# samiazirar/mvtracker

Hardware: AMD Instinct MI355X
Metric: query-points*frames/sec, 4-view 24-frame 512x512 @1024 queries (higher is better)
Workload: dtype bf16; 1 GPU; c3: 4-view synthetic 24-frame 512x512, 1024 queries, bf16 (configs[2], the metric's config); 4-view 24-frame 512x512, 1024 queries per GPU, corr K=16 x 4 levels, iters=4, 3 windows, random-init weights (seeded recipe); queries_total=1024, parallelism=query-shard x1, frame_store=bf16 rows

## Files before the change

### mvtracker_amd/csrc/block_fused.hip

```cpp
#include "common.h"
#include <stdlib.h>

namespace {

typedef __bf16 bf16x8 __attribute__((ext_vector_type(8)));
typedef __bf16 bf16x4 __attribute__((ext_vector_type(4)));
typedef unsigned u32x4 __attribute__((ext_vector_type(4)));
typedef unsigned u32x2 __attribute__((ext_vector_type(2)));

__device__ __forceinline__ void lds_barrier() {
#ifdef MVT_FULL_BARRIERS
  __syncthreads();
#else
  __builtin_amdgcn_fence(__ATOMIC_RELEASE, "workgroup", "local");
  __builtin_amdgcn_s_barrier();
  __builtin_amdgcn_fence(__ATOMIC_ACQUIRE, "workgroup", "local");
#endif
}

constexpr int NT = 512;
constexpr int C = 256;
constexpr int LDX = C + 8;
template <int NMB> struct Cfg {
  static constexpr int BM = 32 * NMB;
  static constexpr int HC = 256;
  static constexpr int JW = HC / 32;
  static constexpr int NM1 = NMB / (8 / JW);
  static constexpr int LDH = HC + 8;
  static constexpr int LDA = 296;
  static_assert(BM * LDA <= 2 * BM * LDH, "attention tile fits the H buffers");
};
constexpr int YLD = 40;
constexpr int FS = 512;

#ifdef MVT_STAMPS
__device__ unsigned long long mvt_stamp_buf[2 * 8 * 64];
#ifndef MVT_STAMP_SEL
#define MVT_STAMP_SEL true
#endif
#ifndef MVT_STAMP_WG1
#define MVT_STAMP_WG1 100
#endif
#define STAMP(i)                                                                                                  \
  do {                                                                                                            \
    __builtin_amdgcn_sched_barrier(0);                                                                            \
    unsigned long long t_;                                                                                        \
    asm volatile("s_memtime %0\n\ts_waitcnt lgkmcnt(0)" : "=s"(t_)::"memory");                                    \
    __builtin_amdgcn_sched_barrier(0);                                                                            \
    if (lane == 0 && MVT_STAMP_SEL && (bx == 0 || bx == MVT_STAMP_WG1) && by == 0 && bz == 0)  \
      mvt_stamp_buf[((bx ? 1 : 0) * 8 + wave) * 64 + (i)] = t_;                                                   \
  } while (0)
#else
#define STAMP(i) \
  do {           \
  } while (0)
#endif

#if defined(MVT_STAMPS) && defined(MVT_ASTAMPS)
#define ASTAMP(i)                                       \
  do {                                                  \
    const int wave = threadIdx.x >> 6;                  \
    const int bx = blockIdx.x, by = blockIdx.y, bz = blockIdx.z; \
    STAMP(i);                                           \
  } while (0)
#else
#define ASTAMP(i) \
  do {            \
  } while (0)
#endif

struct BlockArgs {
  float* x;
  int ldx;
  const float* att;
  int ldatt, Ko;
  const unsigned short* wo;
  const float* bo;
  int ldwo;
  const unsigned short* w1;
  const float* b1;
  const unsigned short* w2;
  const float* b2;
  int ldw1, ldw2, H;
  mvt_block_next next[MVT_BLOCK_MAX_NEXT];
  int n_next;
  int att_bf16;
  long long M;
  float* ws;
  const unsigned short* aq;
  const unsigned short* ak;
  const unsigned short* av;
  int ldaq, ldakv, S, nkeys, bmv;
  const float* parts;
  int nsplit;
  const float* tokx;
  const unsigned short* win;
  const float* bin;
  const float* virt;
  int ldtok;
  long long Mp;
  const float* t_coords;
  const float* t_fcorr;
  const float* t_ffeats;
  const float* t_maskvis;
  const float* t_pos;
  const float* t_time;
  int t_E, t_Fc, t_Cf, t_D;
  const float* c_ws;
  const float* c_b2;
  float* c_x;
  int c_ldx, c_nch;
  mvt_block_next c_kv;
  mvt_block_next c_next;
};

typedef float f32x2 __attribute__((ext_vector_type(2)));
__device__ __forceinline__ f32x2 gelu_tanh_pk(f32x2 x) {
  const f32x2 c0 = {-2.3022082f, -2.3022082f}, c1 = {-0.10294324f, -0.10294324f}, one = {1.0f, 1.0f};
// ... 304 lines not shown
        }
#pragma unroll
        for (int db = 0; db < 2; ++db) {
          const unsigned short* vr = (db * 32 + r < DHA) ? &vimg[(db * 32 + r) * LDVA + 16 * sk + 4 * h] : zrow + 16 * sk + 4 * h;
          const u32x2 a0 = *reinterpret_cast<const u32x2*>(vr), a1 = *reinterpret_cast<const u32x2*>(vr + 8);
          const bf16x8 va = __builtin_bit_cast(bf16x8, (u32x4){a0[0], a0[1], a1[0], a1[1]});
          oacc[db] = __builtin_amdgcn_mfma_f32_32x32x16_bf16(va, pb, oacc[db], 0, 0, 0);
        }
      }
    }
    __builtin_amdgcn_sched_barrier(0);
    ASTAMP(51 + 2 * mb);
    const float lt = pair_sum(ps);
    const float inv = 1.0f / lt;
    if (qi >= nq) continue;
#pragma unroll
    for (int db = 0; db < 2; ++db) {
#pragma unroll
      for (int gq = 0; gq < 4; ++gq) {
        const int d = db * 32 + 8 * gq + 4 * h;
        if (d < DHA) {
          f32x4 t;
#pragma unroll
          for (int e = 0; e < 4; ++e) t[e] = oacc[db][4 * gq + e] * inv;
          *reinterpret_cast<u32x2*>(&As[(arow0 + qi) * lda + hd * DHA + d]) = __builtin_bit_cast(u32x2, __builtin_convertvector(t, bf16x4));
        }
      }
    }
  }
}

template <int NMB>
__device__ __forceinline__ void ln_to_lds(const f32x16 (&v)[NMB], unsigned short* Xs, float* st, int wave, int lane, float eps,
                                          const float* lnw, const float* lnb, float (&ms)[NMB][2], bool have) {
  constexpr int BM = 32 * NMB;
  const int r = lane & 31, h = lane >> 5;
  f32x4 gw[4], gb[4];
  if (lnw) {
#pragma unroll
    for (int g = 0; g < 4; ++g) {
      gw[g] = *reinterpret_cast<const f32x4*>(lnw + wave * 32 + 8 * g + 4 * h);
      gb[g] = *reinterpret_cast<const f32x4*>(lnb + wave * 32 + 8 * g + 4 * h);
    }
  }
  if (!have) {
#pragma unroll
    for (int mb = 0; mb < NMB; ++mb) {
      float s1 = 0.f, s2 = 0.f;
#pragma unroll
      for (int e = 0; e < 16; ++e) {
        s1 += v[mb][e];
        s2 = fmaf(v[mb][e], v[mb][e], s2);
      }
      s1 += __shfl_xor(s1, 32, 64);
      s2 += __shfl_xor(s2, 32, 64);
      if (h == 0) {
        st[(wave * BM + mb * 32 + r) * 2] = s1;
        st[(wave * BM + mb * 32 + r) * 2 + 1] = s2;
      }
    }
    lds_barrier();
#pragma unroll
    for (int mb = 0; mb < NMB; ++mb) {
      float s1 = 0.f, s2 = 0.f;
#pragma unroll
      for (int w = 0; w < 8; ++w) {
        s1 += st[(w * BM + mb * 32 + r) * 2];
        s2 += st[(w * BM + mb * 32 + r) * 2 + 1];
      }
      const float mean = s1 / (float)C;
      ms[mb][0] = mean;
      ms[mb][1] = fmaxf(s2 / (float)C - mean * mean, 0.f);
    }
  }
#pragma unroll
  for (int mb = 0; mb < NMB; ++mb) {
    const float mean = ms[mb][0];
    const float rstd = 1.0f / sqrtf(ms[mb][1] + eps);
#pragma unroll
    for (int g = 0; g < 4; ++g) {
      const int n = wave * 32 + 8 * g + 4 * h;
      f32x4 o;
#pragma unroll
      for (int e = 0; e < 4; ++e) {
        o[e] = (v[mb][4 * g + e] - mean) * rstd;
        if (lnw) o[e] = o[e] * gw[g][e] + gb[g][e];
      }
      const bf16x4 b = __builtin_convertvector(o, bf16x4);
      *reinterpret_cast<u32x2*>(&Xs[(mb * 32 + r) * LDX + n]) = __builtin_bit_cast(u32x2, b);
    }
  }
  lds_barrier();
}

template <int NMB, int MODE, int ATT>
__global__ __launch_bounds__(NT) void block_fused_bf16(BlockArgs p) {
  using K_ = Cfg<NMB>;
  constexpr int BM = K_::BM, HC = K_::HC, LDH = K_::LDH, LDA = K_::LDA;
  constexpr bool CTX = ATT == 6;
  static_assert(!CTX || (NMB == 2 && MODE == 0), "ATT 6 runs on the 64-row tiles of the point rows");
  constexpr int HSZ = CTX && (64 * LDKV + 1) / 2 > BM * LDH ? (64 * LDKV + 1) / 2 : BM * LDH;
  __shared__ __attribute__((aligned(16))) unsigned short Xs[BM * LDX];
  __shared__ __attribute__((aligned(16))) unsigned short Hs[2][HSZ];
  __shared__ float st[8 * BM * 2];
  __shared__ __attribute__((aligned(16))) float b1s[4 * C];
  __shared__ __attribute__((aligned(16))) float cbs[CTX ? 2 * 288 : 4];

  const int t = threadIdx.x, wave = t >> 6, lane = t & 63;
  const int r = lane & 31, h = lane >> 5;
  int bx = (int)blockIdx.x, by = (int)blockIdx.y, bz = (int)blockIdx.z;
  if constexpr (ATT == 2 || ATT == 3 || ATT == 5 || ATT == 6) {
    const unsigned total = gridDim.x * gridDim.y * gridDim.z;
    if (total % 8 == 0) {
      const unsigned L = blockIdx.x + gridDim.x * (blockIdx.y + gridDim.y * blockIdx.z);
      const unsigned V = (L % 8) * (total / 8) + L / 8;
      bx = (int)(V % gridDim.x);
      by = (int)((V / gridDim.x) % gridDim.y);
      bz = (int)(V / (gridDim.x * gridDim.y));
    }
  }
  static_assert(ATT == 0 || ATT == 5 || MODE != 2, "pass 2 of the split path has no attention");
  static_assert(ATT != 5 || MODE == 2, "ATT 5 = pass 2 on the frame-major tiles of an ATT 2 / ATT 3 pass 1");
  static_assert((MODE != 1 && MODE != 2) || NMB == 1, "the split path runs on 32-row tiles");
  constexpr bool FM = ATT == 2 || ATT == 3 || ATT == 5 || ATT == 6;
  const int bmv = ATT == 1 ? p.bmv : BM;
  const long long m0 = FM ? 0 : (long long)bx * bmv;
  const long long ntok = FM ? p.M / p.S : 0;
  auto grow = [&](int i) -> long long {
    if (FM) {
      const long long tk = (long long)bx * BM + i;
      return tk < ntok ? tk * p.S + (long long)bz : -1;
    }
    const long long m = m0 + i;
    return (i < bmv && m < p.M) ? m : -1;
  };
  const long long rlo = FM ? (long long)bx * BM * p.S : m0;
  const long long rhi = FM ? ((long long)bx * BM + BM) * p.S : m0 + bmv;
  constexpr bool HAS_MLP = MODE == 0 || MODE == 1;
  if (HAS_MLP)
    for (int i = t; i < p.H; i += NT) b1s[i] = p.b1[i];
  const long long ws_tile = FM ? (long long)bz * gridDim.x + bx : (long long)bx;
  const long long ws_ntile = FM ? (long long)gridDim.z * gridDim.x : (long long)gridDim.x;
  auto ws_off = [&](int chunk, int g) -> long long { return ((((long long)chunk * ws_ntile + ws_tile) * 8 + wave) * 4 + g) * 256 + lane * 4; };
  auto active = [&](int q) { return q < p.n_next && rlo < p.next[q].row_hi && rhi > p.next[q].row_lo; };
  bf16x8 wq[PFQ];
  constexpr bool EARLY = NMB == 1 && MODE != 0;
  bool early_have = false;
  const bool outp = MODE != 2 && ATT != 4 && (ATT != 0 || p.att != nullptr);
  const unsigned short* wo_row = p.wo + ((long long)wave * 18 * 64 + lane) * 8;
  const unsigned short* fc1_first = p.w1 + ((long long)(wave % K_::JW) * (C / 16) * 64 + lane) * 8 +
                                    (long long)(MODE == 1 ? by : 0) * K_::JW * (C / 16) * FS;
  auto prefetch_wo = [&]() { fill_wq(wq, wo_row); };
  if (HAS_MLP && !outp) {
    fill_wq(wq, fc1_first);
  } else if (CTX) {
    fill_wq(wq, p.c_kv.w + ((long long)wave * (C / 16) * 64 + lane) * 8);
  } else if (outp) {
    prefetch_wo();
  } else if (EARLY && MODE == 2) {
    const int nb0e = by * 8 + wave;
    if (active(0) && nb0e < (p.next[0].N + 31) / 32) {
      fill_wq(wq, p.next[0].w + ((long long)nb0e * (C / 16) * 64 + lane) * 8);
      early_have = true;
    }
  }

  STAMP(0);
  f32x16 v[NMB];
#pragma unroll
  for (int mb = 0; mb < NMB; ++mb)
#pragma unroll
    for (int e = 0; e < 16; ++e) v[mb][e] = 0.f;

  f32x4 xr[NMB][4];
  auto load_x = [&]() {
    if (ATT == 4 || (MODE == 2 && p.ws)) return;
#pragma unroll
// ... 394 lines not shown
            for (int e = 0; e < 4; ++e) xv[e] += part[mb][g][sidx][e];
          }
#pragma unroll
        for (int e = 0; e < 4; ++e) v[mb][4 * g + e] += xv[e] + p.b2[wave * 32 + 8 * g + 4 * h + e];
      }
  } else if (ATT != 4) {
#pragma unroll
    for (int mb = 0; mb < NMB; ++mb)
#pragma unroll
      for (int g = 0; g < 4; ++g)
#pragma unroll
        for (int e = 0; e < 4; ++e) v[mb][4 * g + e] += xr[mb][g][e];
  }

  auto store_x = [&]() {
#pragma unroll
    for (int mb = 0; mb < NMB; ++mb) {
      const long long m = grow(mb * 32 + r);
      if (m >= 0) {
#pragma unroll
        for (int g = 0; g < 4; ++g) {
          f32x4 o;
#pragma unroll
          for (int e = 0; e < 4; ++e) o[e] = v[mb][4 * g + e];
          *reinterpret_cast<f32x4*>(p.x + m * (long long)p.ldx + wave * 32 + 8 * g + 4 * h) = o;
        }
      }
    }
  };
  STAMP(5);
  float ln_ms[NMB][2];
  if (HAS_MLP) ln_to_lds<NMB>(v, Xs, st, wave, lane, 1e-6f, nullptr, nullptr, ln_ms, false);
  STAMP(6);
  const bool tail_next = MODE == 0 && active(0) && wave < (p.next[0].N + 31) / 32;
  if (HAS_MLP) {
    f32x16 acc2[NMB];
#pragma unroll
    for (int mb = 0; mb < NMB; ++mb)
#pragma unroll
      for (int e = 0; e < 16; ++e) acc2[mb][e] = 0.f;
    constexpr int JW = K_::JW, NM1 = K_::NM1;
    const int jb = wave % JW, mp = wave / JW;
    const int nchunk = p.H / HC;
    const unsigned short* w1row = p.w1 + ((long long)jb * (C / 16) * 64 + lane) * 8;
    const unsigned short* w2row = p.w2 + ((long long)wave * (p.H / 16) * 64 + lane) * 8;
    static_assert(HC / 16 == PFQ && C / 16 == PFQ, "every GEMM segment is exactly one queue length");
    const unsigned short* tail = tail_next ? p.next[0].w + ((long long)wave * (C / 16) * 64 + lane) * 8 : w1row;
    const int c_lo = MODE == 1 ? by : 0, c_hi = MODE == 1 ? c_lo + 1 : nchunk;
#pragma unroll 1
    for (int c = c_lo; c < c_hi; ++c) {
      unsigned short* Hb = Hs[c & 1];
      f32x16 ha[NM1];
#pragma unroll
      for (int i = 0; i < NM1; ++i)
#pragma unroll
        for (int e = 0; e < 16; ++e) ha[i][e] = 0.f;
      STAMP(8 + 5 * c);
      gemm_wq<C / 16, NM1>(ha, wq, w1row + (long long)c * JW * (C / 16) * FS, w2row + (long long)c * (HC / 16) * FS, &Xs[r * LDX + 8 * h], LDX,
                           NM1 * mp);
      STAMP(9 + 5 * c);
#pragma unroll
      for (int i = 0; i < NM1; ++i) {
#pragma unroll
        for (int g = 0; g < 4; ++g) {
          const f32x4 bq = *reinterpret_cast<const f32x4*>(&b1s[c * HC + jb * 32 + 8 * g + 4 * h]);
          f32x4 o;
#ifdef MVT_ABL_NOGELU
#pragma unroll
          for (int e = 0; e < 4; ++e) o[e] = ha[i][4 * g + e] + bq[e];
#else
#pragma unroll
          for (int e = 0; e < 4; e += 2) {
            const f32x2 y = gelu_tanh_pk((f32x2){ha[i][4 * g + e] + bq[e], ha[i][4 * g + e + 1] + bq[e + 1]});
            o[e] = y[0];
            o[e + 1] = y[1];
          }
#endif
          const bf16x4 b = __builtin_convertvector(o, bf16x4);
          *reinterpret_cast<u32x2*>(&Hb[((NM1 * mp + i) * 32 + r) * LDH + jb * 32 + 8 * g + 4 * h]) = __builtin_bit_cast(u32x2, b);
        }
// ... 7 lines not shown
    }
    if (MODE == 1) {
#pragma unroll
      for (int mb = 0; mb < NMB; ++mb) {
        const long long m = grow(mb * 32 + r);
        if (m < 0) continue;
#pragma unroll
        for (int g = 0; g < 4; ++g) {
          f32x4 a4, x4;
#pragma unroll
          for (int e = 0; e < 4; ++e) {
            a4[e] = acc2[mb][4 * g + e];
            x4[e] = v[mb][4 * g + e];
          }
          *reinterpret_cast<f32x4*>(p.ws + ws_off(by + 1, g)) = a4;
          if (by == 0) *reinterpret_cast<f32x4*>(p.ws + ws_off(0, g)) = x4;
        }
      }
      return;
    }
#pragma unroll
    for (int mb = 0; mb < NMB; ++mb)
#pragma unroll
      for (int g = 0; g < 4; ++g)
#pragma unroll
        for (int e = 0; e < 4; ++e) v[mb][4 * g + e] += acc2[mb][4 * g + e] + p.b2[wave * 32 + 8 * g + 4 * h + e];
  }
  STAMP(30);
  if (MODE == 0 || ATT == 4 || (p.ws && by == 0)) store_x();
  STAMP(31);

  bool have = tail_next || early_have;
  bool have_ms = false;
#pragma unroll
  for (int q = 0; q < MVT_BLOCK_MAX_NEXT; ++q) {
    if (q >= p.n_next) break;
    if (!active(q)) continue;
    const mvt_block_next nx = p.next[q];
    lds_barrier();
    for (int i = t; i < nx.N; i += NT) b1s[i] = nx.b[i];
    STAMP(32 + 8 * q);
    ln_to_lds<NMB>(v, Xs, st, wave, lane, nx.eps, nx.lnw, nx.lnb, ln_ms, have_ms);
    have_ms = true;
    STAMP(33 + 8 * q);
    const int nblocks = (nx.N + 31) / 32;
    auto nrow_of = [&](int nb) { return nx.w + ((long long)nb * (C / 16) * 64 + lane) * 8; };
    const int nb0 = MODE == 2 ? by * 8 + wave : wave, nbstep = MODE == 2 ? 8 * (int)gridDim.y : 8;
    if (nb0 < nblocks && !have) fill_wq(wq, nrow_of(nb0));
    const int qn = q + 1 < MVT_BLOCK_MAX_NEXT ? q + 1 : MVT_BLOCK_MAX_NEXT - 1;
    const unsigned short* chain = nullptr;
    if ((MODE == 0 || MODE == 3) && q + 1 < MVT_BLOCK_MAX_NEXT && active(q + 1) && wave < (p.next[qn].N + 31) / 32)
      chain = p.next[qn].w + ((long long)wave * (C / 16) * 64 + lane) * 8;
    have = chain != nullptr && wave < nblocks;
    for (int nb = nb0; nb < nblocks; nb += nbstep) {
      f32x16 acc[NMB];
#pragma unroll
      for (int mb = 0; mb < NMB; ++mb)
#pragma unroll
        for (int e = 0; e < 16; ++e) acc[mb][e] = 0.f;
      gemm_wq<C / 16, NMB>(acc, wq, nrow_of(nb), nb + nbstep < nblocks ? nrow_of(nb + nbstep) : (chain ? chain : nrow_of(nb)), &Xs[r * LDX + 8 * h], LDX, 0);
      STAMP(34 + 8 * q + (nb - nb0) / nbstep);
      if (nx.y_bf16 && nb * 32 + 31 < nx.N && (nx.ldy & 7) == 0 && ((uintptr_t)nx.y & 15) == 0) {
        unsigned short* tile = &Hs[0][0] + wave * (NMB * 32 * YLD);
        __builtin_amdgcn_fence(__ATOMIC_SEQ_CST, "wavefront");
#pragma unroll
        for (int mb = 0; mb < NMB; ++mb)
#pragma unroll
          for (int g = 0; g < 4; ++g) {
            f32x4 o;
// ... 32 lines not shown
        }
      }
    }
    STAMP(39 + 8 * q);
  }
  STAMP(63);
}

__global__ void pack_frag_kernel(const unsigned short* __restrict__ w, int ld, int N, int K, unsigned short* __restrict__ out) {
  const long long total = (long long)((N + 31) / 32) * (K / 16) * 64;
  for (long long i = blockIdx.x * (long long)blockDim.x + threadIdx.x; i < total; i += (long long)gridDim.x * blockDim.x) {
    const int lane = (int)(i & 63);
    const long long f = i >> 6;
    const int ks = (int)(f % (K / 16));
    const int nb = (int)(f / (K / 16));
    const int n = nb * 32 + (lane & 31), k = ks * 16 + 8 * (lane >> 5);
    u32x4 v = (u32x4){0u, 0u, 0u, 0u};
    if (n < N) v = *reinterpret_cast<const u32x4*>(w + (long long)n * ld + k);
    *reinterpret_cast<u32x4*>(out + i * 8) = v;
  }
}

}

#ifdef MVT_STAMPS
extern "C" int mvt_debug_read_stamps(unsigned long long* host) {
  return hipMemcpyFromSymbol(host, HIP_SYMBOL(mvt_stamp_buf), sizeof(unsigned long long) * 2 * 8 * 64) == hipSuccess ? MVT_OK : MVT_ERR_HIP_BASE;
}
extern "C" int mvt_debug_clear_stamps() {
  static unsigned long long z[2 * 8 * 64];
  return hipMemcpyToSymbol(HIP_SYMBOL(mvt_stamp_buf), z, sizeof(z)) == hipSuccess ? MVT_OK : MVT_ERR_HIP_BASE;
}
#endif

extern "C" int mvt_pack_frag_bf16(const unsigned short* w, int ld, int N, int K, unsigned short* out, void* stream) {
  MVT_REQUIRE(w && out && N > 0 && K > 0 && K % 16 == 0 && ld % 8 == 0 && ld >= K);
  MVT_REQUIRE(((uintptr_t)w % 16 == 0) && ((uintptr_t)out % 16 == 0));
  const long long total = (long long)((N + 31) / 32) * (K / 16) * 64;
  hipLaunchKernelGGL(pack_frag_kernel, dim3((unsigned)mvt_cdiv(total, 256)), dim3(256), 0, mvt_stream(stream), w, ld, N, K, out);
  return mvt_launch_status();
}

extern "C" int mvt_block_fused_bf16(float* x, int ldx, const void* att, int att_bf16, int ldatt, int Ko, const unsigned short* wo, int ldwo,
                                    const float* bo, const unsigned short* w1, int ldw1, const float* b1, const unsigned short* w2,
                                    int ldw2, const float* b2, int H, const mvt_block_next* next, int n_next, long long M, int Cc,
                                    float* workspace, void* stream) {
  MVT_REQUIRE(x && w1 && b1 && w2 && b2 && M > 0 && Cc == C && H > 0 && H % 256 == 0 && H <= 4 * C);
  MVT_REQUIRE(ldx % 4 == 0 && ldx >= C);
  MVT_REQUIRE(!att || (wo && bo && Ko == 288 && ldatt % 4 == 0 && ldatt >= Ko));
  MVT_REQUIRE(n_next >= 0 && n_next <= MVT_BLOCK_MAX_NEXT && (n_next == 0 || next));
  MVT_REQUIRE(((uintptr_t)x % 16 == 0) && ((uintptr_t)att % 16 == 0) && ((uintptr_t)wo % 16 == 0) && ((uintptr_t)w1 % 16 == 0) &&
              ((uintptr_t)w2 % 16 == 0));
  BlockArgs a{};
  a.x = x; a.ldx = ldx; a.att = (const float*)att; a.att_bf16 = att_bf16 ? 1 : 0; a.ldatt = ldatt; a.Ko = Ko; a.wo = wo; a.bo = bo; a.ldwo = ldwo;
  a.w1 = w1; a.b1 = b1; a.w2 = w2; a.b2 = b2; a.ldw1 = ldw1; a.ldw2 = ldw2; a.H = H; a.M = M; a.n_next = n_next;
  for (int q = 0; q < n_next; ++q) {
    const mvt_block_next& nx = next[q];
    MVT_REQUIRE(nx.w && nx.b && nx.y && nx.N > 0 && nx.N <= 4 * C && nx.ldy % 4 == 0 && nx.ldy >= nx.N);
    MVT_REQUIRE(nx.y_bf16 == 0 || nx.y_bf16 == 1);
    MVT_REQUIRE((nx.lnw == nullptr) == (nx.lnb == nullptr) && ((uintptr_t)nx.lnw % 16 == 0) && ((uintptr_t)nx.lnb % 16 == 0) && ((uintptr_t)nx.w % 16 == 0) && ((uintptr_t)nx.y % 16 == 0));
    MVT_REQUIRE(nx.row_lo >= 0 && (nx.row_hi == 0 || nx.row_hi > nx.row_lo));
    a.next[q] = nx;
    if (nx.row_hi == 0) a.next[q].row_hi = M;
  }
  static const char* force = getenv("MVT_BLOCK_NMB");
  const int nmb = force ? atoi(force) : (M >= 4096 ? 2 : 1);
  static const bool no_split = getenv("MVT_BLOCK_NOSPLIT") != nullptr;
  a.ws = workspace;
  if (nmb == 2) {
    hipLaunchKernelGGL((block_fused_bf16<2, 0, 0>), dim3((unsigned)mvt_cdiv(M, 64)), dim3(NT), 0, mvt_stream(stream), a);
  } else if (workspace && !no_split && M <= 2048 && M % 32 == 0) {
    MVT_REQUIRE((uintptr_t)workspace % 16 == 0);
    const unsigned tiles = (unsigned)mvt_cdiv(M, 32);
    hipLaunchKernelGGL((block_fused_bf16<1, 1, 0>), dim3(tiles, (unsigned)(H / 256)), dim3(NT), 0, mvt_stream(stream), a);
    int maxblk = 1;
    for (int q = 0; q < n_next; ++q) maxblk = (next[q].N + 31) / 32 > maxblk ? (next[q].N + 31) / 32 : maxblk;
    const unsigned slices = n_next ? (unsigned)mvt_cdiv(maxblk, 8) : 1u;
    hipLaunchKernelGGL((block_fused_bf16<1, 2, 0>), dim3(tiles, slices), dim3(NT), 0, mvt_stream(stream), a);
  } else {
    hipLaunchKernelGGL((block_fused_bf16<1, 0, 0>), dim3((unsigned)mvt_cdiv(M, 32)), dim3(NT), 0, mvt_stream(stream), a);
  }
  return mvt_launch_status();
}

extern "C" int mvt_attn_block_fused_bf16(float* x, int ldx, const mvt_block_attn* attn, const unsigned short* wo, const float* bo,
                                         const unsigned short* w1, const float* b1, const unsigned short* w2, const float* b2, int H,
                                         const mvt_block_next* next, int n_next, long long M, int Cc, float* workspace, void* stream) {
  MVT_REQUIRE(x && attn && wo && bo && w1 && b1 && w2 && b2 && M > 0 && Cc == C && H > 0 && H % 256 == 0 && H <= 4 * C);
  MVT_REQUIRE(ldx % 4 == 0 && ldx >= C && n_next >= 0 && n_next <= MVT_BLOCK_MAX_NEXT && (n_next == 0 || next));
  MVT_REQUIRE(attn->heads == 6 && attn->dim_head == DHA && attn->S >= 1 && M % attn->S == 0);
  MVT_REQUIRE(attn->kind == MVT_ATTN_PARTIALS || (attn->kind == MVT_ATTN_FRAME_CTX && attn->q && attn->ldq % 8 == 0 && attn->ldq >= 288) ||
              (attn->q && attn->k && attn->v && attn->ldq % 8 == 0 && attn->ldkv % 8 == 0 && attn->ldq >= 288 && attn->ldkv >= 288));
  MVT_REQUIRE(((uintptr_t)x % 16 == 0) && ((uintptr_t)wo % 16 == 0) && ((uintptr_t)w1 % 16 == 0) && ((uintptr_t)w2 % 16 == 0));
  MVT_REQUIRE(((uintptr_t)attn->q % 16 == 0) && ((uintptr_t)attn->k % 16 == 0) && ((uintptr_t)attn->v % 16 == 0));
  BlockArgs a{};
  a.x = x; a.ldx = ldx; a.att = nullptr; a.Ko = 288; a.wo = wo; a.bo = bo; a.ldwo = 288;
  a.w1 = w1; a.b1 = b1; a.w2 = w2; a.b2 = b2; a.ldw1 = C; a.ldw2 = H; a.H = H; a.M = M; a.n_next = n_next; a.ws = workspace;
  a.aq = attn->q; a.ak = attn->k; a.av = attn->v; a.ldaq = attn->ldq; a.ldakv = attn->ldkv; a.S = attn->S; a.nkeys = attn->n_keys;
  for (int q = 0; q < n_next; ++q) {
    const mvt_block_next& nx = next[q];
    MVT_REQUIRE(nx.w && nx.b && nx.y && nx.N > 0 && nx.N <= 4 * C && nx.ldy % 4 == 0 && nx.ldy >= nx.N);
    MVT_REQUIRE((nx.y_bf16 == 0 || nx.y_bf16 == 1) && (nx.lnw == nullptr) == (nx.lnb == nullptr) && ((uintptr_t)nx.lnw % 16 == 0) && ((uintptr_t)nx.lnb % 16 == 0));
    MVT_REQUIRE(((uintptr_t)nx.w % 16 == 0) && ((uintptr_t)nx.y % 16 == 0) && nx.row_lo >= 0 && (nx.row_hi == 0 || nx.row_hi > nx.row_lo));
    a.next[q] = nx;
    if (nx.row_hi == 0) a.next[q].row_hi = M;
  }
  const int S = attn->S;
  if (attn->kind == MVT_ATTN_TIME) {
    MVT_REQUIRE(S <= 32 && !workspace);
    static const bool small_tiles = !(getenv("MVT_TIME_NMB1") && atoi(getenv("MVT_TIME_NMB1")) == 0);
    if (small_tiles && mvt_cdiv(M, (32 / S) * S) <= 256) {
      a.bmv = (32 / S) * S;
      hipLaunchKernelGGL((block_fused_bf16<1, 0, 1>), dim3((unsigned)mvt_cdiv(M, a.bmv)), dim3(NT), 0, mvt_stream(stream), a);
      return mvt_launch_status();
    }
    a.bmv = (64 / S) * S;
    hipLaunchKernelGGL((block_fused_bf16<2, 0, 1>), dim3((unsigned)mvt_cdiv(M, a.bmv)), dim3(NT), 0, mvt_stream(stream), a);
  } else if (attn->kind == MVT_ATTN_PARTIALS) {
    MVT_REQUIRE(attn->partials && attn->n_splits >= 1 && attn->n_splits <= MVT_ATTN_NSPLIT && attn->n_keys == 64 && M == 64LL * S);
    MVT_REQUIRE(workspace && (uintptr_t)workspace % 16 == 0 && M <= 2048 && (uintptr_t)attn->partials % 16 == 0);
    a.parts = attn->partials; a.nsplit = attn->n_splits;
    const unsigned tiles = (unsigned)mvt_cdiv(M, 32);
    a.S = S;
    hipLaunchKernelGGL((block_fused_bf16<1, 1, 3>), dim3(2, (unsigned)(H / 256), (unsigned)S), dim3(NT), 0, mvt_stream(stream), a);
    int maxblk = 1;
    for (int q = 0; q < n_next; ++q) maxblk = (next[q].N + 31) / 32 > maxblk ? (next[q].N + 31) / 32 : maxblk;
    const unsigned slices = n_next ? (unsigned)mvt_cdiv(maxblk, 8) : 1u;
    (void)tiles;
    if (!attn->defer_pass2)
      hipLaunchKernelGGL((block_fused_bf16<1, 2, 5>), dim3(2, slices, (unsigned)S), dim3(NT), 0, mvt_stream(stream), a);
  } else if (attn->kind == MVT_ATTN_FRAME) {
    MVT_REQUIRE(attn->n_keys >= 1 && attn->n_keys <= 64);
    const long long ntok = M / S;
    static const bool small_tiles = !(getenv("MVT_FRAME_NMB1") && atoi(getenv("MVT_FRAME_NMB1")) == 0);
    if (ntok * S >= 4096 && small_tiles && mvt_cdiv(ntok, 32) * S <= 256) {
      MVT_REQUIRE(!workspace);
      hipLaunchKernelGGL((block_fused_bf16<1, 0, 2>), dim3((unsigned)mvt_cdiv(ntok, 32), 1, (unsigned)S), dim3(NT), 0, mvt_stream(stream), a);
    } else if (ntok * S >= 4096) {
      MVT_REQUIRE(!workspace);
      hipLaunchKernelGGL((block_fused_bf16<2, 0, 2>), dim3((unsigned)mvt_cdiv(ntok, 64), 1, (unsigned)S), dim3(NT), 0, mvt_stream(stream), a);
    } else {
      MVT_REQUIRE(workspace && (uintptr_t)workspace % 16 == 0 && M <= 2048 && ntok % 32 == 0);
      hipLaunchKernelGGL((block_fused_bf16<1, 1, 2>), dim3((unsigned)(ntok / 32), (unsigned)(H / 256), (unsigned)S), dim3(NT), 0,
                         mvt_stream(stream), a);
      int maxblk = 1;
      for (int q = 0; q < n_next; ++q) maxblk = (next[q].N + 31) / 32 > maxblk ? (next[q].N + 31) / 32 : maxblk;
      const unsigned slices = n_next ? (unsigned)mvt_cdiv(maxblk, 8) : 1u;
      if (!attn->defer_pass2)
        hipLaunchKernelGGL((block_fused_bf16<1, 2, 5>), dim3((unsigned)(ntok / 32), slices, (unsigned)S), dim3(NT), 0, mvt_stream(stream), a);
    }
  } else if (attn->kind == MVT_ATTN_FRAME_CTX) {
    const mvt_block_ctx* cx = attn->ctx;
    const long long ntok = M / S;
    MVT_REQUIRE(cx && attn->n_keys == 64 && ntok * S >= 4096 && !workspace && !attn->defer_pass2);
    MVT_REQUIRE(cx->ws && cx->b2 && cx->x && cx->chunks >= 1 && cx->chunks <= 4 && cx->ldx % 4 == 0 && cx->ldx >= C);
    MVT_REQUIRE(((uintptr_t)cx->ws % 16 == 0) && ((uintptr_t)cx->b2 % 16 == 0) && ((uintptr_t)cx->x % 16 == 0));
    MVT_REQUIRE(cx->kv.w && cx->kv.b && cx->kv.N == 2 * 288 && (cx->kv.lnw == nullptr) == (cx->kv.lnb == nullptr));
    MVT_REQUIRE(((uintptr_t)cx->kv.w % 16 == 0) && ((uintptr_t)cx->kv.lnw % 16 == 0) && ((uintptr_t)cx->kv.lnb % 16 == 0));
    const unsigned tiles = (unsigned)mvt_cdiv(ntok, 64);
    if (cx->next.w) {
      const mvt_block_next& nx = cx->next;
      MVT_REQUIRE(nx.b && nx.y && nx.N > 0 && nx.N <= 4 * C && nx.ldy % 4 == 0 && nx.ldy >= nx.N && (nx.y_bf16 == 0 || nx.y_bf16 == 1));
      MVT_REQUIRE((nx.lnw == nullptr) == (nx.lnb == nullptr) && ((uintptr_t)nx.lnw % 16 == 0) && ((uintptr_t)nx.lnb % 16 == 0));
      MVT_REQUIRE(((uintptr_t)nx.w % 16 == 0) && ((uintptr_t)nx.y % 16 == 0) && (nx.N + 31) / 32 <= 8 * (int)tiles);
    }
    a.c_ws = cx->ws; a.c_b2 = cx->b2; a.c_x = cx->x; a.c_ldx = cx->ldx; a.c_nch = cx->chunks; a.c_kv = cx->kv; a.c_next = cx->next;
    hipLaunchKernelGGL((block_fused_bf16<2, 0, 6>), dim3(tiles, 1, (unsigned)S), dim3(NT), 0, mvt_stream(stream), a);
  } else {
    return MVT_ERR_ARG;
  }
  return mvt_launch_status();
}

extern "C" int mvt_input_proj_bf16(const float* tokens, int ldtok, int token_dim, long long Mp, const unsigned short* win, const float* bin,
                                   const float* virtual_tokens, int S, float* x, int ldx, const mvt_block_next* next, int n_next, long long M,
                                   int Cc, void* stream) {
  MVT_REQUIRE(tokens && win && bin && virtual_tokens && x && next && n_next >= 1 && n_next <= MVT_BLOCK_MAX_NEXT && Cc == C);
  MVT_REQUIRE(M > 0 && Mp >= 0 && Mp <= M && S >= 1 && (M - Mp) % S == 0 && token_dim >= 1 && token_dim <= 37 * 16 && ldtok >= token_dim);
  MVT_REQUIRE(ldtok % 4 == 0 && ldx % 4 == 0 && ldx >= C && ((uintptr_t)tokens % 16 == 0) && ((uintptr_t)win % 16 == 0) && ((uintptr_t)x % 16 == 0));
  BlockArgs a{};
  a.x = x; a.ldx = ldx; a.M = M; a.n_next = n_next; a.H = 4 * C; a.ws = nullptr; a.S = S;
  a.tokx = tokens; a.ldtok = ldtok; a.win = win; a.bin = bin; a.virt = virtual_tokens; a.Mp = Mp;
  for (int q = 0; q < n_next; ++q) {
    const mvt_block_next& nx = next[q];
    MVT_REQUIRE(nx.w && nx.b && nx.y && nx.N > 0 && nx.N <= 4 * C && nx.ldy % 4 == 0 && nx.ldy >= nx.N);
    MVT_REQUIRE((nx.lnw == nullptr) == (nx.lnb == nullptr) && ((uintptr_t)nx.lnw % 16 == 0) && ((uintptr_t)nx.lnb % 16 == 0) && ((uintptr_t)nx.w % 16 == 0) && ((uintptr_t)nx.y % 16 == 0));
    MVT_REQUIRE(nx.row_lo >= 0 && (nx.row_hi == 0 || nx.row_hi > nx.row_lo) && (nx.y_bf16 == 0 || nx.y_bf16 == 1));
    a.next[q] = nx;
    if (nx.row_hi == 0) a.next[q].row_hi = M;
  }
  hipLaunchKernelGGL((block_fused_bf16<2, 3, 4>), dim3((unsigned)mvt_cdiv(M, 64)), dim3(NT), 0, mvt_stream(stream), a);
  return mvt_launch_status();
}

extern "C" int mvt_token_input_proj_bf16(const float* coords, const float* fcorr, int Fc, const float* ffeats, int Cf, const float* mask_vis,
                                         const float* pos, const float* time_embed, int n_tracks, int S, int E,
                                         const unsigned short* win, const float* bin, const float* virtual_tokens, float* x, int ldx,
                                         const mvt_block_next* next, int n_next, long long M, int Cc, void* stream) {
  MVT_REQUIRE(coords && fcorr && ffeats && mask_vis && pos && time_embed && win && bin && virtual_tokens && x && next);
  MVT_REQUIRE(n_next >= 1 && n_next <= MVT_BLOCK_MAX_NEXT && Cc == C && n_tracks > 0 && S >= 1 && E > 0 && E % 2 == 0 && Fc > 0 && Cf > 0);
  const int D = 3 * E + 3 + Fc + Cf + 2;
  const long long Mp = (long long)n_tracks * S;
  MVT_REQUIRE(D <= 37 * 16 && M >= Mp && (M - Mp) % S == 0 && ldx % 4 == 0 && ldx >= C);
  MVT_REQUIRE(((uintptr_t)win % 16 == 0) && ((uintptr_t)x % 16 == 0));
  BlockArgs a{};
  a.x = x; a.ldx = ldx; a.M = M; a.n_next = n_next; a.H = 4 * C; a.ws = nullptr; a.S = S;
  a.tokx = nullptr; a.win = win; a.bin = bin; a.virt = virtual_tokens; a.Mp = Mp;
  a.t_coords = coords; a.t_fcorr = fcorr; a.t_ffeats = ffeats; a.t_maskvis = mask_vis; a.t_pos = pos; a.t_time = time_embed;
  a.t_E = E; a.t_Fc = Fc; a.t_Cf = Cf; a.t_D = D;
  for (int q = 0; q < n_next; ++q) {
    const mvt_block_next& nx = next[q];
    MVT_REQUIRE(nx.w && nx.b && nx.y && nx.N > 0 && nx.N <= 4 * C && nx.ldy % 4 == 0 && nx.ldy >= nx.N);
    MVT_REQUIRE((nx.lnw == nullptr) == (nx.lnb == nullptr) && ((uintptr_t)nx.lnw % 16 == 0) && ((uintptr_t)nx.lnb % 16 == 0) && ((uintptr_t)nx.w % 16 == 0) && ((uintptr_t)nx.y % 16 == 0));
    MVT_REQUIRE(nx.row_lo >= 0 && (nx.row_hi == 0 || nx.row_hi > nx.row_lo) && (nx.y_bf16 == 0 || nx.y_bf16 == 1));
    a.next[q] = nx;
    if (nx.row_hi == 0) a.next[q].row_hi = M;
  }
  hipLaunchKernelGGL((block_fused_bf16<2, 3, 4>), dim3((unsigned)mvt_cdiv(M, 64)), dim3(NT), 0, mvt_stream(stream), a);
  return mvt_launch_status();
}

extern "C" int mvt_ln_proj_bf16(const float* x, int ldx, const mvt_block_next* next, int n_next, long long M, int Cc, void* stream) {
  MVT_REQUIRE(x && next && n_next >= 1 && n_next <= MVT_BLOCK_MAX_NEXT && M > 0 && Cc == C && ldx % 4 == 0 && ldx >= C);
  MVT_REQUIRE((uintptr_t)x % 16 == 0);
  BlockArgs a{};
  a.x = const_cast<float*>(x); a.ldx = ldx; a.M = M; a.n_next = n_next; a.H = 4 * C; a.ws = nullptr;
  int maxblk = 1;
  for (int q = 0; q < n_next; ++q) {
    const mvt_block_next& nx = next[q];
    MVT_REQUIRE(nx.w && nx.b && nx.y && nx.N > 0 && nx.N <= 4 * C && nx.ldy % 4 == 0 && nx.ldy >= nx.N);
    MVT_REQUIRE((nx.lnw == nullptr) == (nx.lnb == nullptr) && ((uintptr_t)nx.lnw % 16 == 0) && ((uintptr_t)nx.lnb % 16 == 0) && ((uintptr_t)nx.w % 16 == 0) && ((uintptr_t)nx.y % 16 == 0));
    MVT_REQUIRE(nx.row_lo >= 0 && (nx.row_hi == 0 || nx.row_hi > nx.row_lo) && (nx.y_bf16 == 0 || nx.y_bf16 == 1));
    a.next[q] = nx;
    if (nx.row_hi == 0) a.next[q].row_hi = M;
    maxblk = (nx.N + 31) / 32 > maxblk ? (nx.N + 31) / 32 : maxblk;
  }
  if (M >= 4096)
    hipLaunchKernelGGL((block_fused_bf16<2, 3, 0>), dim3((unsigned)mvt_cdiv(M, 64)), dim3(NT), 0, mvt_stream(stream), a);
  else
    hipLaunchKernelGGL((block_fused_bf16<1, 2, 0>), dim3((unsigned)mvt_cdiv(M, 32), (unsigned)mvt_cdiv(maxblk, 8)), dim3(NT), 0,
                       mvt_stream(stream), a);
  return mvt_launch_status();
}
```

### mvtracker_amd/csrc/common.h

```cpp
#pragma once
#include <hip/hip_runtime.h>
#include <stdint.h>

#include "../../include/mvtracker_hip.h"

typedef float f32x4 __attribute__((ext_vector_type(4)));
typedef float f32x16 __attribute__((ext_vector_type(16)));

#define MVT_WAVE 64

#define MVT_REQUIRE(cond) \
  do {                    \
    if (!(cond)) return MVT_ERR_ARG; \
  } while (0)

static inline int mvt_launch_status() {
  hipError_t e = hipGetLastError();
  return e == hipSuccess ? MVT_OK : MVT_ERR_HIP_BASE + (int)e;
}

static inline hipStream_t mvt_stream(void* s) { return (hipStream_t)s; }

static inline long long mvt_cdiv(long long a, long long b) { return (a + b - 1) / b; }

__device__ __forceinline__ float mvt_gelu_tanh(float x) {
  const float k2 = 2.0f * 0.7978845608028654f * (x + 0.044715f * x * x * x);
  return x * __builtin_amdgcn_rcpf(1.0f + __expf(-k2));
}

__device__ __forceinline__ float mvt_gelu_erf(float x) { return 0.5f * x * (1.0f + erff(x * 0.7071067811865476f)); }

__device__ __forceinline__ float mvt_act(float x, int act) {
  switch (act) {
    case MVT_ACT_RELU: return fmaxf(x, 0.0f);
    case MVT_ACT_GELU_TANH: return mvt_gelu_tanh(x);
    case MVT_ACT_GELU_ERF: return mvt_gelu_erf(x);
    default: return x;
  }
}

__device__ __forceinline__ f32x4 mvt_unproject_point(const float* __restrict__ K, const float* __restrict__ E, int x, int y, float st, float d) {
  float px = ((float)x + 0.5f) * st - 0.5f, py = ((float)y + 0.5f) * st - 0.5f;
  float cx = (K[0] * px + K[1] * py + K[2]) * d;
  float cy = (K[3] * px + K[4] * py + K[5]) * d;
  float cz = (K[6] * px + K[7] * py + K[8]) * d;
  f32x4 o;
  o[0] = E[0] * cx + E[1] * cy + E[2] * cz + E[3];
  o[1] = E[4] * cx + E[5] * cy + E[6] * cz + E[7];
  o[2] = E[8] * cx + E[9] * cy + E[10] * cz + E[11];
  o[3] = 0.f;
  return o;
}

__device__ __forceinline__ unsigned short mvt_bf16_bits(float v) { return __builtin_bit_cast(unsigned short, (__bf16)v); }
__device__ __forceinline__ f32x4 load_act4(const float* base, long long off, int is_bf16) {
  if (!is_bf16) return *reinterpret_cast<const f32x4*>(base + off);
// ... 63 lines not shown
```

### mvtracker_amd/csrc/updater.hip

```cpp
#include "common.h"
#include <stdlib.h>

namespace {

inline long long align256(long long b) { return (b + 255) & ~255LL; }

struct Layout {
  long long tok, qkv_a, qkv_b, qp, att, split_ws, attn_ws, vrep, h1, h2, total;
  int ldh;
};

constexpr int H_ = 256, HEADS = 6, DH_ = 48, INNER = HEADS * DH_, NV = 64, MLP = 1024, OUT = 131;

inline Layout layout(long long n, long long S, long long G = 1) {
  const long long Mp = n * S, Mv = G * NV * S, M = Mp + Mv;
  Layout L{};
  long long o = 0;
  auto take = [&](long long bytes) { const long long at = o; o += align256(bytes); return at; };
  L.tok = take(M * H_ * 4);
  L.qkv_a = take(M * 3 * INNER * 2);
  L.qkv_b = take(M * 3 * INNER * 2);
  L.qp = take(Mp * INNER * 2);
  L.att = take(M * INNER * 2);
  L.split_ws = take((MLP / 256 + 1) * Mv * H_ * 4);
// ... 98 lines not shown
  const bool grouped = G > 1;
  const bool fuse_time = (w->fuse_attention & 1) && S <= 32, fuse_p2v = (w->fuse_attention & 2) && !grouped,
             fuse_vs = (w->fuse_attention & 4) && !grouped;
  long long* prow = nullptr;
  long long* vrow = nullptr;
  int* nvs = nullptr;
  struct Tables {
    long long* a = nullptr;
    int* b = nullptr;
    ~Tables() { free(a); free(b); }
  } tables;
  if (grouped) {
    tables.a = (long long*)malloc(sizeof(long long) * 2 * G);
    tables.b = (int*)malloc(sizeof(int) * G);
    if (!tables.a || !tables.b) return MVT_ERR_ARG;
    prow = tables.a;
    vrow = tables.a + G;
    nvs = tables.b;
    long long off = 0;
    for (int g = 0; g < G; ++g) {
      prow[g] = off * S;
      vrow[g] = (long long)g * NV * S;
      nvs[g] = NV;
      off += gn[g];
    }
  }
  const float* vtokens = w->virtual_tokens;
  if (grouped) {
    float* vrep = (float*)(base + L.vrep);
    MVT_TRY(mvt_broadcast_rows_repeat(w->virtual_tokens, vrep, H_, NV, 1, H_, G, stream));
    vtokens = vrep;
  }
  static const bool small_m = !(getenv("MVT_FRAME_NMB1") && atoi(getenv("MVT_FRAME_NMB1")) == 0);
  const bool small_form = small_m && (long long)n * S >= 4096 && (long long)((n + 31) / 32) * S <= 256;
  const bool fold_vs = (w->fuse_attention & 32) && !grouped && fuse_p2v && fuse_vs && (long long)n * S >= 4096 && !small_form && MLP / 256 <= 4 &&
                       8 * ((n + 63) / 64) >= (3 * INNER + 31) / 32;

  {
    const mvt_block_next nx = next_of(w->time_blk[0].qkv, qkv, ld3, 0, 0);
    if (!x) {
      MVT_REQUIRE(w->token_dim <= 592 && w->input_frag.K == 592);
      MVT_TRY(mvt_token_input_proj_bf16(ti->coords, ti->fcorr, ti->Fc, ti->ffeats, ti->Cf, ti->mask_vis, ti->pos, ti->time_embed, n, S, ti->E,
                                        w->input_frag.w, w->input_frag.b, vtokens, tok, H_, &nx, 1, M, H_, stream));
    } else if (w->input_frag.w && w->token_dim <= 592 && w->input_frag.K == 592) {
      MVT_TRY(mvt_input_proj_bf16(x, ldx, w->token_dim, Mp, w->input_frag.w, w->input_frag.b, vtokens, S, tok, H_, &nx, 1, M, H_,
                                  stream));
    } else {
      MVT_TRY(mvt_gemm_bf16(x, ldx, w->input_transform.w, nullptr, w->input_transform.ldw, w->input_transform.b, nullptr, 0, tok, H_, (int)Mp,
                            H_, w->token_dim, MVT_ACT_NONE, 0, stream));
      MVT_TRY(grouped ? mvt_broadcast_rows_repeat(w->virtual_tokens, vt, H_, NV, S, H_, G, stream)
                      : mvt_broadcast_rows(w->virtual_tokens, vt, H_, NV, S, H_, stream));
      MVT_TRY(mvt_ln_proj_bf16(tok, H_, &nx, 1, M, H_, stream));
    }
  }
  for (int i = 0; i < w->depth; ++i) {
    const bool last = i + 1 == w->depth;
    const mvt_updater_block &tb = w->time_blk[i], &v2p = w->v2p[i], &vs = w->vself[i], &p2v = w->p2v[i];
    {
      const mvt_block_next nx[3] = {next_of(v2p.kv, qkv + INNER, ld3, 0, Mp, v2p.ctx_ln_w, v2p.ctx_ln_b, 1e-5f),
                                    next_of(p2v.q, qp, INNER, 0, Mp), next_of(v2p.q, qkv, ld3, Mp, M)};
      if (fuse_time) {
        MVT_TRY(attn_block(tb, tok, M, MVT_ATTN_TIME, qkv, ld3, qkv + INNER, qkv + 2 * INNER, S, nx, 3, nullptr));
      } else {
        MVT_TRY(mvt_attention_bf16(qkv, ld3, S, 1, qkv + INNER, qkv + 2 * INNER, ld3, S, 1, att, INNER, n + G * NV, S, S, HEADS, DH_, BF,
                                   nullptr, stream));
        MVT_TRY(block(tb, tok, M, att, nx, 3, nullptr));
      }
// ... 106 lines not shown
```

Measured before the change: 1.038 million query-points*frames/s.

## Deal next-layer projection column blocks across all waves in fused block kernel

Instead of running each follow-on projection (the next layer's QKV and similar) one after another with a barrier each, the fused block kernel now builds one list of 32-column blocks across all active projections and deals them round-robin to the eight waves. Up to two distinct LayerNorm images are kept in LDS, the second in a new Xs2 buffer, and each wave writes bf16 results through a per-wave tile. This is meant to cut the per-projection barriers and the idle waves when a projection has fewer column blocks than waves. In exchange it costs extra LDS, a bigger bias buffer and more register pressure. A host-side planner turns the path on only when alignment and size conditions hold, and an environment variable turns it off.

After: 1.053 million query-points*frames/s (median of 6 runs). 1.01x the previous value.

```diff
diff --git a/mvtracker_amd/csrc/block_fused.hip b/mvtracker_amd/csrc/block_fused.hip
--- a/mvtracker_amd/csrc/block_fused.hip
+++ b/mvtracker_amd/csrc/block_fused.hip
@@ -31,6 +31,7 @@
   static_assert(BM * LDA <= 2 * BM * LDH, "attention tile fits the H buffers");
 };
 constexpr int YLD = 40;
+constexpr int NBIAS_DEAL = 4 * 256 + 256;
 constexpr int FS = 512;
 
 #ifdef MVT_STAMPS
@@ -84,6 +85,7 @@
   int ldw1, ldw2, H;
   mvt_block_next next[MVT_BLOCK_MAX_NEXT];
   int n_next;
+  int deal, deal_img[MVT_BLOCK_MAX_NEXT], deal_rep[2];
   int att_bf16;
   long long M;
   float* ws;
@@ -454,7 +456,7 @@
 
 template <int NMB>
 __device__ __forceinline__ void ln_to_lds(const f32x16 (&v)[NMB], unsigned short* Xs, float* st, int wave, int lane, float eps,
-                                          const float* lnw, const float* lnb, float (&ms)[NMB][2], bool have) {
+                                          const float* lnw, const float* lnb, float (&ms)[NMB][2], bool have, bool sync = true) {
   constexpr int BM = 32 * NMB;
   const int r = lane & 31, h = lane >> 5;
   f32x4 gw[4], gb[4];
@@ -512,7 +514,31 @@
       *reinterpret_cast<u32x2*>(&Xs[(mb * 32 + r) * LDX + n]) = __builtin_bit_cast(u32x2, b);
     }
   }
-  lds_barrier();
+  if (sync) lds_barrier();
+}
+
+template <int NM, class GR>
+__device__ __forceinline__ void proj_store(const f32x16 (&acc)[NM], unsigned short* tile, const float* bias, unsigned short* yb,
+                                           int ldy, long long row_lo, long long row_hi, GR grow, int lane) {
+  const int r = lane & 31, h = lane >> 5;
+  __builtin_amdgcn_fence(__ATOMIC_SEQ_CST, "wavefront");
+#pragma unroll
+  for (int mb = 0; mb < NM; ++mb)
+#pragma unroll
+    for (int g = 0; g < 4; ++g) {
+      f32x4 o;
+#pragma unroll
+      for (int e = 0; e < 4; ++e) o[e] = acc[mb][4 * g + e] + bias[8 * g + 4 * h + e];
+      *reinterpret_cast<u32x2*>(&tile[(mb * 32 + r) * YLD + 8 * g + 4 * h]) = __builtin_bit_cast(u32x2, __builtin_convertvector(o, bf16x4));
+    }
+  __builtin_amdgcn_fence(__ATOMIC_SEQ_CST, "wavefront");
+#pragma unroll
+  for (int k = 0; k < NM * 2; ++k) {
+    const int pc = lane + 64 * k, row = pc >> 2, c = pc & 3;
+    const long long m = grow(row);
+    if (m >= row_lo && m < row_hi)
+      *reinterpret_cast<u32x4*>(yb + m * (long long)ldy + c * 8) = *reinterpret_cast<const u32x4*>(&tile[row * YLD + c * 8]);
+  }
 }
 
 template <int NMB, int MODE, int ATT>
@@ -525,7 +551,10 @@
   __shared__ __attribute__((aligned(16))) unsigned short Xs[BM * LDX];
   __shared__ __attribute__((aligned(16))) unsigned short Hs[2][HSZ];
   __shared__ float st[8 * BM * 2];
-  __shared__ __attribute__((aligned(16))) float b1s[4 * C];
+  constexpr bool DEAL = MODE == 0 || MODE == 3;
+  constexpr int NBIAS = DEAL ? NBIAS_DEAL : 4 * C;
+  __shared__ __attribute__((aligned(16))) unsigned short Xs2[DEAL ? BM * LDX : 8];
+  __shared__ __attribute__((aligned(16))) float b1s[NBIAS];
   __shared__ __attribute__((aligned(16))) float cbs[CTX ? 2 * 288 : 4];
 
   const int t = threadIdx.x, wave = t >> 6, lane = t & 63;
@@ -565,6 +594,18 @@
   const long long ws_ntile = FM ? (long long)gridDim.z * gridDim.x : (long long)gridDim.x;
   auto ws_off = [&](int chunk, int g) -> long long { return ((((long long)chunk * ws_ntile + ws_tile) * 8 + wave) * 4 + g) * 256 + lane * 4; };
   auto active = [&](int q) { return q < p.n_next && rlo < p.next[q].row_hi && rhi > p.next[q].row_lo; };
+  static_assert(MVT_BLOCK_MAX_NEXT == 3, "three projections in the packed scalar and in the selects of section 3");
+  unsigned d_pack = 0;
+  if constexpr (DEAL) {
+#pragma unroll
+    for (int q = 0; q < MVT_BLOCK_MAX_NEXT; ++q) {
+      const long long lo = p.next[q].row_lo, hi = p.next[q].row_hi;
+      const unsigned nb = (unsigned)(p.next[q].N >> 5) & 0xFFu, im = p.deal_img[q] ? 1u << 25 : 1u << 24;
+      const bool on = (q < p.n_next) & (rlo < hi) & (rhi > lo);
+      d_pack |= ((nb << (8 * q)) | im) & (0u - (unsigned)on);
+    }
+    d_pack |= p.deal ? 1u << 26 : 0u;
+  }
   bf16x8 wq[PFQ];
   constexpr bool EARLY = NMB == 1 && MODE != 0;
   bool early_have = false;
@@ -1025,7 +1066,37 @@
   float ln_ms[NMB][2];
   if (HAS_MLP) ln_to_lds<NMB>(v, Xs, st, wave, lane, 1e-6f, nullptr, nullptr, ln_ms, false);
   STAMP(6);
-  const bool tail_next = MODE == 0 && active(0) && wave < (p.next[0].N + 31) / 32;
+  const int wv = __builtin_amdgcn_readfirstlane(wave);
+  int d_nb[MVT_BLOCK_MAX_NEXT], d_first[MVT_BLOCK_MAX_NEXT];
+  int d_T = 0;
+#pragma unroll
+  for (int q = 0; q < MVT_BLOCK_MAX_NEXT; ++q) {
+    d_nb[q] = (int)((d_pack >> (8 * q)) & 0xFFu);
+    d_first[q] = d_T;
+    d_T += d_nb[q];
+  }
+  const bool d_im0 = (d_pack >> 24) & 1u, d_im1 = (d_pack >> 25) & 1u;
+  const bool dealt = DEAL && ((d_pack >> 26) & 1u) && (d_nb[0] > 0) + (d_nb[1] > 0) + (d_nb[2] > 0) >= 2;
+  auto item_q = [&](int i, int& nb) {
+    int q = 0;
+    nb = i;
+#pragma unroll
+    for (int qq = 0; qq + 1 < MVT_BLOCK_MAX_NEXT; ++qq)
+      if (q == qq && nb >= d_nb[qq]) {
+        nb -= d_nb[qq];
+        q = qq + 1;
+      }
+    return q;
+  };
+  auto item_wrow = [&](int i) {
+    int nb;
+    const int q = item_q(i, nb);
+    const unsigned short* w = q == 0 ? p.next[0].w : q == 1 ? p.next[1].w : p.next[2].w;
+    return w + ((long long)nb * (C / 16) * 64 + lane) * 8;
+  };
+  const int d_full = (d_T >> 3) + (wv < (d_T & 7) ? 1 : 0);
+  const int d_head = d_full > 0 ? wv : -1;
+  const bool tail_next = !dealt && MODE == 0 && active(0) && wave < (p.next[0].N + 31) / 32;
   if (HAS_MLP) {
     f32x16 acc2[NMB];
 #pragma unroll
@@ -1038,7 +1109,7 @@
     const unsigned short* w1row = p.w1 + ((long long)jb * (C / 16) * 64 + lane) * 8;
     const unsigned short* w2row = p.w2 + ((long long)wave * (p.H / 16) * 64 + lane) * 8;
     static_assert(HC / 16 == PFQ && C / 16 == PFQ, "every GEMM segment is exactly one queue length");
-    const unsigned short* tail = tail_next ? p.next[0].w + ((long long)wave * (C / 16) * 64 + lane) * 8 : w1row;
+    const unsigned short* tail = dealt && d_head >= 0 ? item_wrow(d_head) : tail_next ? p.next[0].w + ((long long)wave * (C / 16) * 64 + lane) * 8 : w1row;
     const int c_lo = MODE == 1 ? by : 0, c_hi = MODE == 1 ? c_lo + 1 : nchunk;
 #pragma unroll 1
     for (int c = c_lo; c < c_hi; ++c) {
@@ -1112,9 +1183,64 @@
 
   bool have = tail_next || early_have;
   bool have_ms = false;
+  if (dealt) {
+    if constexpr (DEAL) {
+      lds_barrier();
+#pragma unroll
+      for (int q = 0; q < MVT_BLOCK_MAX_NEXT; ++q)
+        if (d_nb[q] > 0)
+          for (int i = t; i < p.next[q].N; i += NT) b1s[d_first[q] * 32 + i] = p.next[q].b[i];
+      if (MODE != 0 && d_head >= 0) fill_wq(wq, item_wrow(d_head));
+      STAMP(32);
+      if (d_im0) {
+        const int q0 = p.deal_rep[0];
+        const float* lnw = q0 == 0 ? p.next[0].lnw : q0 == 1 ? p.next[1].lnw : p.next[2].lnw;
+        const float* lnb = q0 == 0 ? p.next[0].lnb : q0 == 1 ? p.next[1].lnb : p.next[2].lnb;
+        const float eps = q0 == 0 ? p.next[0].eps : q0 == 1 ? p.next[1].eps : p.next[2].eps;
+        ln_to_lds<NMB>(v, Xs, st, wave, lane, eps, lnw, lnb, ln_ms, false, !d_im1);
+      }
+      if (d_im1) {
+        const int q1 = p.deal_rep[1];
+        const float* lnw = q1 == 1 ? p.next[1].lnw : p.next[2].lnw;
+        const float* lnb = q1 == 1 ? p.next[1].lnb : p.next[2].lnb;
+        const float eps = q1 == 1 ? p.next[1].eps : p.next[2].eps;
+        ln_to_lds<NMB>(v, Xs2, st, wave, lane, eps, lnw, lnb, ln_ms, d_im0, true);
+      }
+      STAMP(33);
+      unsigned short* tile = &Hs[0][0] + wave * (NMB * 32 * YLD);
+      auto item_y = [&](int q, int nb) {
+        float* y = q == 0 ? p.next[0].y : q == 1 ? p.next[1].y : p.next[2].y;
+        return reinterpret_cast<unsigned short*>(y) + nb * 32;
+      };
+      auto item_ldy = [&](int q) { return q == 0 ? p.next[0].ldy : q == 1 ? p.next[1].ldy : p.next[2].ldy; };
+      auto item_lo = [&](int q) { return q == 0 ? p.next[0].row_lo : q == 1 ? p.next[1].row_lo : p.next[2].row_lo; };
+      auto item_hi = [&](int q) { return q == 0 ? p.next[0].row_hi : q == 1 ? p.next[1].row_hi : p.next[2].row_hi; };
+      auto item_xs = [&](int q) {
+        const int im = q == 0 ? p.deal_img[0] : q == 1 ? p.deal_img[1] : p.deal_img[2];
+        return (im ? &Xs2[0] : &Xs[0]) + r * LDX + 8 * h;
+      };
+#pragma unroll 1
+      for (int k = 0; k < d_full; ++k) {
+        const int i = wv + 8 * k;
+        int nb;
+        const int q = item_q(i, nb);
+        const int inext = k + 1 < d_full ? i + 8 : -1;
+        const unsigned short* row = item_wrow(i);
+        f32x16 acc[NMB];
+#pragma unroll
+        for (int mb = 0; mb < NMB; ++mb)
+#pragma unroll
+          for (int e = 0; e < 16; ++e) acc[mb][e] = 0.f;
+        gemm_wq<C / 16, NMB>(acc, wq, row, inext >= 0 ? item_wrow(inext) : row, item_xs(q), LDX, 0);
+        STAMP(34 + (k < 4 ? k : 4));
+        proj_store<NMB>(acc, tile, &b1s[32 * i], item_y(q, nb), item_ldy(q), item_lo(q), item_hi(q), grow, lane);
+      }
+      STAMP(39);
+    }
+  }
 #pragma unroll
   for (int q = 0; q < MVT_BLOCK_MAX_NEXT; ++q) {
-    if (q >= p.n_next) break;
+    if (q >= p.n_next || dealt) break;
     if (!active(q)) continue;
     const mvt_block_next nx = p.next[q];
     lds_barrier();
@@ -1213,6 +1339,31 @@
   return hipMemcpyToSymbol(HIP_SYMBOL(mvt_stamp_buf), z, sizeof(z)) == hipSuccess ? MVT_OK : MVT_ERR_HIP_BASE;
 }
 #endif
+
+static inline int proj_seq_switch() {
+  const char* e = getenv("MVT_PROJ_SEQ");
+  return e && atoi(e) != 0;
+}
+static void plan_deal(BlockArgs& a) {
+  a.deal = 0;
+  if (proj_seq_switch() || a.n_next == 0) return;
+  int nimg = 0, total = 0;
+  for (int q = 0; q < a.n_next; ++q) {
+    const mvt_block_next& nx = a.next[q];
+    if (!nx.y_bf16 || (nx.N & 31) || (nx.ldy & 7) || ((uintptr_t)nx.y & 15)) return;
+    int im = -1;
+    for (int qq = 0; qq < q && im < 0; ++qq)
+      if (a.next[qq].lnw == nx.lnw && a.next[qq].lnb == nx.lnb && a.next[qq].eps == nx.eps) im = a.deal_img[qq];
+    if (im < 0) {
+      if (nimg == 2) return;
+      im = nimg++;
+      a.deal_rep[im] = q;
+    }
+    a.deal_img[q] = im;
+    total += nx.N;
+  }
+  if (total <= NBIAS_DEAL) a.deal = 1;
+}
 
 extern "C" int mvt_pack_frag_bf16(const unsigned short* w, int ld, int N, int K, unsigned short* out, void* stream) {
   MVT_REQUIRE(w && out && N > 0 && K > 0 && K % 16 == 0 && ld % 8 == 0 && ld >= K);
@@ -1244,6 +1395,7 @@
     a.next[q] = nx;
     if (nx.row_hi == 0) a.next[q].row_hi = M;
   }
+  plan_deal(a);
   static const char* force = getenv("MVT_BLOCK_NMB");
   const int nmb = force ? atoi(force) : (M >= 4096 ? 2 : 1);
   static const bool no_split = getenv("MVT_BLOCK_NOSPLIT") != nullptr;
@@ -1286,6 +1438,7 @@
     a.next[q] = nx;
     if (nx.row_hi == 0) a.next[q].row_hi = M;
   }
+  plan_deal(a);
   const int S = attn->S;
   if (attn->kind == MVT_ATTN_TIME) {
     MVT_REQUIRE(S <= 32 && !workspace);
@@ -1314,7 +1467,7 @@
     MVT_REQUIRE(attn->n_keys >= 1 && attn->n_keys <= 64);
     const long long ntok = M / S;
     static const bool small_tiles = !(getenv("MVT_FRAME_NMB1") && atoi(getenv("MVT_FRAME_NMB1")) == 0);
-    if (ntok * S >= 4096 && small_tiles && mvt_cdiv(ntok, 32) * S <= 256) {
+    if (small_tiles && mvt_frame_small_tiles(ntok, S)) {
       MVT_REQUIRE(!workspace);
       hipLaunchKernelGGL((block_fused_bf16<1, 0, 2>), dim3((unsigned)mvt_cdiv(ntok, 32), 1, (unsigned)S), dim3(NT), 0, mvt_stream(stream), a);
     } else if (ntok * S >= 4096) {
@@ -1370,6 +1523,7 @@
     a.next[q] = nx;
     if (nx.row_hi == 0) a.next[q].row_hi = M;
   }
+  plan_deal(a);
   hipLaunchKernelGGL((block_fused_bf16<2, 3, 4>), dim3((unsigned)mvt_cdiv(M, 64)), dim3(NT), 0, mvt_stream(stream), a);
   return mvt_launch_status();
 }
@@ -1397,6 +1551,7 @@
     a.next[q] = nx;
     if (nx.row_hi == 0) a.next[q].row_hi = M;
   }
+  plan_deal(a);
   hipLaunchKernelGGL((block_fused_bf16<2, 3, 4>), dim3((unsigned)mvt_cdiv(M, 64)), dim3(NT), 0, mvt_stream(stream), a);
   return mvt_launch_status();
 }
@@ -1416,6 +1571,7 @@
     if (nx.row_hi == 0) a.next[q].row_hi = M;
     maxblk = (nx.N + 31) / 32 > maxblk ? (nx.N + 31) / 32 : maxblk;
   }
+  plan_deal(a);
   if (M >= 4096)
     hipLaunchKernelGGL((block_fused_bf16<2, 3, 0>), dim3((unsigned)mvt_cdiv(M, 64)), dim3(NT), 0, mvt_stream(stream), a);
   else
diff --git a/mvtracker_amd/csrc/common.h b/mvtracker_amd/csrc/common.h
--- a/mvtracker_amd/csrc/common.h
+++ b/mvtracker_amd/csrc/common.h
@@ -22,6 +22,8 @@
 static inline hipStream_t mvt_stream(void* s) { return (hipStream_t)s; }
 
 static inline long long mvt_cdiv(long long a, long long b) { return (a + b - 1) / b; }
+
+static inline bool mvt_frame_small_tiles(long long ntok, long long S) { return ntok * S >= 4096 && mvt_cdiv(ntok, 32) * S <= 256; }
 
 __device__ __forceinline__ float mvt_gelu_tanh(float x) {
   const float k2 = 2.0f * 0.7978845608028654f * (x + 0.044715f * x * x * x);
diff --git a/mvtracker_amd/csrc/updater.hip b/mvtracker_amd/csrc/updater.hip
--- a/mvtracker_amd/csrc/updater.hip
+++ b/mvtracker_amd/csrc/updater.hip
@@ -154,7 +154,7 @@
     vtokens = vrep;
   }
   static const bool small_m = !(getenv("MVT_FRAME_NMB1") && atoi(getenv("MVT_FRAME_NMB1")) == 0);
-  const bool small_form = small_m && (long long)n * S >= 4096 && (long long)((n + 31) / 32) * S <= 256;
+  const bool small_form = small_m && mvt_frame_small_tiles(n, S);
   const bool fold_vs = (w->fuse_attention & 32) && !grouped && fuse_p2v && fuse_vs && (long long)n * S >= 4096 && !small_form && MLP / 256 <= 4 &&
                        8 * ((n + 63) / 64) >= (3 * INNER + 31) / 32;
 
```
